# KrishnaswamyLab/MELD

Hardware: AMD Instinct MI355X
Metric: cells/sec through MELD.fit_transform (kNN+Chebyshev) (higher is better)
Workload: dtype f64

## Files before the change

include/meld_hip.h:

```cpp
#ifndef MELD_HIP_H
#define MELD_HIP_H

#include <stddef.h>
#include <stdint.h>

#ifdef __cplusplus
extern "C" {
#endif

#define MELD_OK 0
#define MELD_ERR_INVALID (-1)
#define MELD_ERR_UNSUPPORTED (-2)
#define MELD_ERR_HIP (-3)

typedef void* meld_stream_t;

int meld_abi_version(void);
const char* meld_last_error(void);
int meld_device_count(void);


int meld_knn_padded_dim(int d);
int meld_knn_tile_refs(void);
int meld_knn_block_queries(void);
// ... 274 lines not shown
                       const double* state, double* nrm2, meld_stream_t stream);
int meld_scale_f64(const double* x, double a, double* r, int64_t n, meld_stream_t stream);
int meld_axpby_f64(double a, const double* x, double b, double* y, int64_t n, double* nrm2,
                   meld_stream_t stream);

typedef struct meld_pt_layout {
  const int32_t* blk_row;
  const int32_t* blk_ntile;
  const int32_t* blk_ndist;
  const int32_t* seg;
  const int32_t* list_cols;
  const double* pval;
  const uint32_t* pidx;
  int32_t nb;
  const float* pval32;
  int64_t stream_len;
  const uint16_t* cdesc;
} meld_pt_layout_t;
int meld_pt_geometry(int* consumer_waves, int* rows_max, int* tile_cols, int* tiles_max);
int meld_pt_num_blocks(int64_t n_rows);
int64_t meld_pt_seg_len(int nb);
int64_t meld_pt_stream_len(int64_t nnz, int nb);
int64_t meld_pt_desc_len(int nb);
int meld_pt_build(const int64_t* rowptr, const int32_t* col, const double* val, int64_t n_rows, int64_t n_cols,
                  int64_t col_base, int symmetric, const meld_pt_layout_t* layout,
                  uint32_t* codes , int32_t* status, meld_stream_t stream);

int meld_rccl_available(void);
int meld_rccl_unique_id(void* id_host);
int meld_rccl_comm_create(const void* id_host, int world, int rank, void** comm);
int meld_rccl_comm_destroy(void* comm);
int meld_rccl_all_gather(void* comm, const void* send, void* recv, size_t bytes_per_rank, meld_stream_t stream);
int meld_rccl_all_reduce_sum_f64(void* comm, double* buf, size_t count, meld_stream_t stream);
int meld_cheby_run(void* comm, const meld_laplacian_t* L, int64_t rows_pad, int64_t row_begin, int p, double* t_a, double* t_b,
                   double* r, const double* coeffs, int n_coef, double alpha2, double beta2, int* last, meld_stream_t stream);
int meld_lanczos_steps_sharded(void* comm, const meld_laplacian_t* L, int64_t rows_pad, int64_t row_begin, double* v0, double* v1,
                               double* v2, double* state, double* acc, double* alphas, double* betas, int it_begin, int n_iter,
                               meld_stream_t stream);

int meld_kmeans_max_blocks(void);
int meld_kmeans_assign(const double* X, int64_t n, int d, const double* centroids, int k, int32_t* labels,
                       double* part_sum, double* part_cnt, double* part_inertia, int n_blocks, meld_stream_t stream);

int meld_kmeans_wide_max_d(void);
int meld_kmeans_wide_max_k(void);
int meld_kmeans_wide_assign(const double* Y, int64_t ldy, int64_t n, int d, const double* centres, int k, double* centre_norms,
// ... 141 lines not shown
```

meld_amd/_lib.py:

```python
from __future__ import annotations

from ._options import is_set, opt

import ctypes as C
import os

_HERE = os.path.dirname(os.path.abspath(__file__))
LIB_NAME = "libmeld_hip.so"
LIB_PATH = os.path.join(_HERE, LIB_NAME)

_i32, _i64, _f64, _sz, _ptr = C.c_int, C.c_int64, C.c_double, C.c_size_t, C.c_void_p

SIGNATURES = {
    "meld_abi_version": (_i32, []),
    "meld_last_error": (C.c_char_p, []),
    "meld_device_count": (_i32, []),
    "meld_knn_padded_dim": (_i32, [_i32]),
    "meld_knn_tile_refs": (_i32, []),
    "meld_knn_block_queries": (_i32, []),
    "meld_knn_row_capacity": (_i32, [_i32]),
    "meld_col_sums_f64": (_i32, [_ptr, _i64, _i32, _ptr, _ptr]),
    "meld_col_stats_temp_bytes": (_sz, [_i32]),
    "meld_col_stats_f64": (_i32, [_ptr, _i64, _i32, _ptr, _ptr, _ptr, _ptr, _sz, _ptr]),
    "meld_knn_prepare_refs": (_i32, [_ptr, _i64, _i32, _ptr, _i32, _ptr, _ptr, _ptr, _ptr]),
# ... 94 lines not shown
    "meld_csr_rows_sort_merge_sums": (_i32, [_ptr, _i64, _ptr, _ptr, _ptr, _ptr, _i32, _f64, _f64, _ptr, _ptr]),
    "meld_csr_compact_rows_anisotropy": (_i32, [_ptr, _i64, _ptr, _ptr, _ptr, _ptr, _ptr, _f64, _ptr, _ptr]),
    "meld_csr_compact_rows_sums": (_i32, [_ptr, _i64, _ptr, _ptr, _ptr, _ptr, _f64, _ptr, _ptr]),
    "meld_csr_row_sums": (_i32, [_ptr, _ptr, _i64, _f64, _ptr, _ptr]),
    "meld_csr_anisotropy": (_i32, [_ptr, _ptr, _ptr, _i64, _ptr, _i64, _f64, _ptr]),
    "meld_csr_anisotropy_degrees": (_i32, [_ptr, _ptr, _ptr, _i64, _ptr, _i64, _f64, _ptr, _ptr]),
    "meld_extend_rows_temp_bytes": (_sz, [_i64, _i64]),
    "meld_extend_rows": (_i32, [_ptr, _ptr, _i64, _i64, _i64, _i64, _ptr, _ptr, _ptr, _ptr, _ptr, _sz, _ptr]),
    "meld_extend_apply": (_i32, [_ptr, _ptr, _ptr, _ptr, _i64, _ptr, _i64, _i32, _ptr, _ptr, _ptr]),
    "meld_spmm_dot_slots": (_i32, []),
    "meld_cheby_step": (_i32, [_ptr, _i32, _ptr, _i64, _ptr, _ptr, _ptr, _f64, _f64, _f64, _f64, _ptr, _ptr]),
    "meld_lanczos_steps": (_i32, [_ptr, _ptr, _ptr, _ptr, _ptr, _ptr, _ptr, _i32, _i32, _ptr, _ptr, _ptr]),
    "meld_lanczos_spmv": (_i32, [_ptr, _ptr, _i64, _ptr, _ptr, _ptr, _ptr, _ptr]),
    "meld_lanczos_alpha": (_i32, [_ptr, _ptr, _ptr, _ptr, _i32, _ptr]),
    "meld_lanczos_axpy": (_i32, [_ptr, _ptr, _i64, _ptr, _ptr, _ptr]),
    "meld_lanczos_beta": (_i32, [_ptr, _ptr, _ptr, _ptr, _i32, _ptr]),
    "meld_lanczos_fold": (_i32, [_ptr, _ptr, _ptr, _ptr, _i32, _ptr]),
    "meld_lanczos_axpy3": (_i32, [_ptr, _ptr, _ptr, _i64, _ptr, _ptr, _ptr]),
    "meld_pt_geometry": (_i32, [_ptr, _ptr, _ptr, _ptr]),
    "meld_pt_num_blocks": (_i32, [_i64]),
    "meld_pt_seg_len": (_i64, [_i32]),
    "meld_pt_stream_len": (_i64, [_i64, _i32]),
    "meld_pt_desc_len": (_i64, [_i32]),
    "meld_pt_build": (_i32, [_ptr, _ptr, _ptr, _i64, _i64, _i64, _i32, _ptr, _ptr, _ptr, _ptr]),
    "meld_cheby_step_wide": (_i32, [_ptr, _i32, _ptr, _i64, _ptr, _ptr, _f64, _f64, _f64, _ptr]),
    "meld_block_max_blocks": (_i32, []),
    "meld_block_gram_f64": (_i32, [_ptr, _i64, _ptr, _i64, _i64, _i32, _ptr, _i32, _ptr, _ptr]),
    "meld_block_rotate_f64": (_i32, [_ptr, _i64, _ptr, _i64, _i32, _ptr, _i64, _ptr]),
    "meld_block_residuals_f64": (_i32, [_ptr, _ptr, _i64, _ptr, _i64, _i32, _ptr, _i32, _ptr, _ptr]),
    "meld_kmeans_max_blocks": (_i32, []),
    "meld_kmeans_assign": (_i32, [_ptr, _i64, _i32, _ptr, _i32, _ptr, _ptr, _ptr, _ptr, _i32, _ptr]),
    "meld_kmeans_wide_max_d": (_i32, []),
    "meld_kmeans_wide_max_k": (_i32, []),
    "meld_kmeans_wide_assign": (_i32, [_ptr, _i64, _i64, _i32, _ptr, _i32, _ptr, _ptr, _ptr, _ptr]),
    "meld_kmeans_wide_sums": (_i32, [_ptr, _i64, _i64, _i32, _ptr, _ptr, _i32, _ptr, _ptr]),
    "meld_scale_f64": (_i32, [_ptr, _f64, _ptr, _i64, _ptr]),
    "meld_axpby_f64": (_i32, [_f64, _ptr, _f64, _ptr, _i64, _ptr, _ptr]),
    "meld_normalize_rows_l1": (_i32, [_ptr, _ptr, _i64, _i32, _ptr]),
    "meld_assign_nearest": (_i32, [_ptr, _i64, _i32, _ptr, _i32, _ptr, _ptr, _ptr, _ptr]),
    "meld_chain_order": (_i32, [_ptr, _i64, _i32, _i32, _ptr, _ptr]),
    "meld_gather_rows_f64": (_i32, [_ptr, _ptr, _i64, _i32, _ptr, _ptr]),
    "meld_frame_max_dims": (_i32, []),
    "meld_cov_sample_f64": (_i32, [_ptr, _i64, _i32, _ptr, _i64, _ptr, _ptr]),
    "meld_rotate_rows_f64": (_i32, [_ptr, _i64, _i32, _ptr, _ptr, _ptr, _ptr]),
    "meld_argsort_u32_temp_bytes": (_sz, [_i64]),
    "meld_argsort_u32": (_i32, [_ptr, _i64, _i32, _ptr, _ptr, _ptr, _sz, _ptr]),
# ... 109 lines not shown
```

meld_amd/csrc/spmm_tiled.hip:

```cpp
#include "common.hpp"

#include <algorithm>
#include <cstdlib>
#include <cstring>

namespace meld {
namespace pt {

constexpr int NW = 12;
constexpr int NL = 4;
constexpr int THREADS = 64 * (NW + NL);
constexpr int RMAX = 4080;
constexpr int SLOTS = RMAX / NW;
constexpr int RPAD = 4096;
constexpr int CP = 1024;
constexpr int CP_BITS = 10;
constexpr int NB = 4;
constexpr int TMAX = 61;
constexpr int SEGW = 64;
constexpr int SEGROWS = 2 * (NW + 1);
constexpr int QW = 8;
constexpr int PADCAP = 64;
constexpr int KMAX = 512;
constexpr int KSLACK = 32;
// ... 428 lines not shown
        d_yy += yv.v[c] * yv.v[c];
      }
      stg<P>(ys, row, a.ld, a.colofs, yv);
      if (a.r != nullptr) stg<P>(a.r, row, a.ld, a.colofs, rl_[q]);
    }
  }
  if (a.dots != nullptr) {
    d_yx = wave_sum(d_yx);
    d_yy = wave_sum(d_yy);
    if (lane == 0) {
      s_dot[0][w] = d_yx;
      s_dot[1][w] = d_yy;
    }
    __syncthreads();
    if (tid < 2) {
      double s = 0.0;
      for (int k = 0; k < NW + NL; ++k) s += s_dot[tid][k];
      atomicAdd(&a.dots[tid * DOT_SLOTS + (b % DOT_SLOTS)], s);
    }
  }
}


__global__ __launch_bounds__(1024) void pt_plan_kernel(const int64_t* __restrict__ rowptr, int64_t n_rows, int nb,
                                                       int32_t* __restrict__ blk_row) {
  const int64_t nnz = rowptr[n_rows];
  for (int b = threadIdx.x; b < nb; b += blockDim.x) {
    const int64_t target = (nnz / nb) * (b + 1) + ((nnz % nb) * (b + 1)) / nb;
    int64_t lo = 0, hi = n_rows;
    while (lo < hi) {
      const int64_t mid = (lo + hi) >> 1;
      if (rowptr[mid] < target) lo = mid + 1; else hi = mid;
    }
    blk_row[b + 1] = (int32_t)((b == nb - 1) ? n_rows : lo);
  }
  __syncthreads();
  if (threadIdx.x == 0) {
    int64_t prev = 0;
    blk_row[0] = 0;
    for (int b = 0; b < nb; ++b) {
      int64_t cut = blk_row[b + 1];
      const int64_t must = n_rows - (int64_t)(nb - 1 - b) * RMAX;
      cut = max(cut, must);
      cut = min(cut, prev + RMAX);
      cut = min(max(cut, prev), n_rows);
      blk_row[b + 1] = (int32_t)cut;
      prev = cut;
    }
  }
}

constexpr int W_ENTRY = 361, W_FAR = 754, W_ROW = 2840;
__global__ __launch_bounds__(256) void pt_row_weight_kernel(const int64_t* __restrict__ rowptr, const int32_t* __restrict__ col,
                                                            int64_t n_rows, int64_t col_base, int win, int32_t* __restrict__ w) {
  const int64_t i = ((int64_t)blockIdx.x * blockDim.x + threadIdx.x) >> 4;
  const int sub = threadIdx.x & 15;
  int far = 0;
  int64_t e0 = 0, e1 = 0;
  if (i < n_rows) {
    e0 = rowptr[i];
    e1 = rowptr[i + 1];
    const int64_t self = col_base + i;
    for (int64_t e = e0 + sub; e < e1; e += 16) {
      const int64_t dlt = (int64_t)col[e] - self;
      far += (dlt > win || dlt < -win) ? 1 : 0;
    }
  }
#pragma unroll
  for (int off = 8; off > 0; off >>= 1) far += __shfl_xor(far, off, 64);
  if (i < n_rows && sub == 0) {
    const int64_t v = (int64_t)W_ENTRY * (e1 - e0) + (int64_t)W_FAR * far + W_ROW;
    w[i] = (int32_t)min(v, (int64_t)0x3fffffff);
  }
}
__global__ __launch_bounds__(1024) void pt_plan_weighted_kernel(const int64_t* __restrict__ wpre, int64_t n_rows, int nb,
                                                                int32_t* __restrict__ blk_row) {
  const int64_t tot = wpre[n_rows];
  for (int b = threadIdx.x; b < nb; b += blockDim.x) {
    const int64_t target = (tot / nb) * (b + 1) + ((tot % nb) * (b + 1)) / nb;
    int64_t lo = 0, hi = n_rows;
    while (lo < hi) {
      const int64_t mid = (lo + hi) >> 1;
      if (wpre[mid] < target) lo = mid + 1; else hi = mid;
    }
    blk_row[b + 1] = (int32_t)((b == nb - 1) ? n_rows : lo);
  }
  __syncthreads();
  if (threadIdx.x == 0) {
    int64_t prev = 0;
    blk_row[0] = 0;
    for (int b = 0; b < nb; ++b) {
      int64_t cut = blk_row[b + 1];
      const int64_t must = n_rows - (int64_t)(nb - 1 - b) * RMAX;
      cut = max(cut, must);
      cut = min(cut, prev + RMAX);
      cut = min(max(cut, prev), n_rows);
      blk_row[b + 1] = (int32_t)cut;
      prev = cut;
    }
  }
}

__device__ __forceinline__ int block_exscan(int v, int* s_wave , int* total) {
  const int lane = threadIdx.x & 63, w = threadIdx.x >> 6;
  int inc = v;
#pragma unroll
  for (int off = 1; off < 64; off <<= 1) {
    const int t = __shfl_up(inc, off, 64);
    if (lane >= off) inc += t;
  }
  __syncthreads();
  if (lane == 63) s_wave[w] = inc;
  __syncthreads();
  if (threadIdx.x == 0) {
    int run = 0;
    for (int k = 0; k < THREADS / 64; ++k) {
      const int t = s_wave[k];
      s_wave[k] = run;
      run += t;
    }
    s_wave[THREADS / 64] = run;
  }
  __syncthreads();
  *total = s_wave[THREADS / 64];
  return s_wave[w] + inc - v;
}

constexpr int GW = 4;
constexpr int GPP = (BP / 32) / GW;
constexpr int GROUPS_MAX = TP_MAX * GPP;
constexpr int GPT = (GROUPS_MAX + THREADS - 1) / THREADS;

__device__ __forceinline__ uint64_t lanes_below(int l) { return ((uint64_t)1 << l) - 1; }

__global__ __launch_bounds__(THREADS) void pt_build_kernel(
    const int64_t* __restrict__ rowptr, const int32_t* __restrict__ col, int64_t n_cols, int64_t col_base, int sym,
    int nb, const int32_t* __restrict__ blk_row, int32_t* __restrict__ blk_ntile, int32_t* __restrict__ blk_ndist,
    int32_t* __restrict__ seg, uint16_t* __restrict__ cdesc, int32_t* __restrict__ list_cols, uint32_t* __restrict__ codes,
    int32_t* __restrict__ status) {
  __shared__ int16_t s_pmap[NPAN_MAX];
  __shared__ uint32_t s_bits[TP_MAX][BP / 32];
  __shared__ int32_t s_gpre[GROUPS_MAX + 1];
  __shared__ int16_t s_cpan[TP_MAX];
  __shared__ int32_t s_cnt[NW][SEGW];
  __shared__ int32_t s_nin[NW];
  __shared__ int s_scan[THREADS / 64 + 1];
  __shared__ int32_t s_rp[RMAX + 1];
  __shared__ int s_ord[SEGW];
  __shared__ int s_tmp[2][SEGW];
  __shared__ int32_t s_len[NW];

  const int tid = threadIdx.x;
  const int lane = tid & 63;
  const int w = tid >> 6;
  const int b = blockIdx.x;
  const int row0 = blk_row[b];
  const int nrows = blk_row[b + 1] - row0;
  const int64_t e0 = rowptr[row0];
  const int64_t e1 = rowptr[row0 + nrows];
  const int npan = (int)((n_cols + BP - 1) / BP);
  const int64_t cb0 = col_base + row0;
  auto in_block = [&](int c) { return sym && (uint64_t)((int64_t)c - cb0) < (uint64_t)nrows; };
  int32_t* segp = seg + (size_t)b * SEGROWS * SEGW;

  for (int i = tid; i < NPAN_MAX; i += THREADS) s_pmap[i] = 0;
  for (int i = tid; i < TP_MAX * (BP / 32); i += THREADS) (&s_bits[0][0])[i] = 0u;
  for (int i = tid; i < NW * SEGW; i += THREADS) (&s_cnt[0][0])[i] = 0;
  for (int i = tid; i <= nrows; i += THREADS) s_rp[i] = (int32_t)(rowptr[row0 + i] - e0);
  for (int i = tid; i < SEGROWS * SEGW; i += THREADS) segp[i] = 0;
  __syncthreads();
  auto write_header = [&](int T_, int ndist_) {
    int32_t* h = segp + (SEGROWS - 1) * SEGW;
    h[2] = row0;
    h[3] = nrows;
    h[4] = T_;
    h[5] = ndist_;
    h[6] = (int32_t)(uint32_t)((uint64_t)e0 & 0xFFFFFFFFu);
    h[7] = (int32_t)(uint32_t)((uint64_t)e0 >> 32);
  };
  if (nrows == 0 || e1 == e0) {
    if (tid == 0) {
      blk_ntile[b] = 0;
      blk_ndist[b] = 0;
      write_header(0, 0);
    }
    return;
  }

  constexpr int MU = 8;
  for (int64_t eb = e0 + tid; eb < e1; eb += (int64_t)MU * THREADS) {
    int c[MU];
#pragma unroll
// ... 19 lines not shown
      if (pn < NPAN_MAX) s_pmap[pn] = f[k] ? (int16_t)(pre++) : (int16_t)-1;
    }
    if (tid == 0) s_scan[0] = total;
  }
  __syncthreads();
  const int tp_all = s_scan[0];
  __syncthreads();

  constexpr int RU = 8;
  const int nmine = (w < NW && nrows > w) ? (nrows - w + NW - 1) / NW : 0;
  const int64_t elast = max(e1 - 1, e0);
  int curs = 0;
  int in_cur = 0;
  int dist_base = 0;
  bool bad_range = false, bad_diag = false;
  const int n_groups_p = max(1, (tp_all + TP_MAX - 1) / TP_MAX);
  for (int pg = 0; pg < n_groups_p; ++pg) {
  const int pbase = pg * TP_MAX;
  const int tp = min(TP_MAX, tp_all - pbase);
  auto panel_slot = [&](int c) -> int {
    const int ci = (int)s_pmap[c >> BP_BITS] - pbase;
    return ((unsigned)ci < (unsigned)TP_MAX) ? ci : -1;
  };
  if (pg > 0) {
    for (int i = tid; i < TP_MAX * (BP / 32); i += THREADS) (&s_bits[0][0])[i] = 0u;
  }
  for (int pn = tid; pn < npan; pn += THREADS) {
    const int ci = (int)s_pmap[pn] - pbase;
    if (s_pmap[pn] >= 0 && (unsigned)ci < (unsigned)TP_MAX) s_cpan[ci] = (int16_t)pn;
  }
  __syncthreads();

  for (int64_t eb = e0 + tid; eb < e1; eb += (int64_t)MU * THREADS) {
    int c[MU];
#pragma unroll
    for (int u = 0; u < MU; ++u) c[u] = col[min(eb + (int64_t)u * THREADS, e1 - 1)];
#pragma unroll
    for (int u = 0; u < MU; ++u) {
      if (in_block(c[u])) continue;
      const int ci = panel_slot(c[u]);
      if (ci >= 0) atomicOr(&s_bits[ci][(c[u] & (BP - 1)) >> 5], 1u << (c[u] & 31));
    }
  }
  __syncthreads();
  int ndist_g;
  {
    const int ngroups = tp * GPP;
    int cntk[GPT], c = 0;
#pragma unroll
// ... 116 lines not shown
          bad_range |= ipos > 0x1FFF;
          codes[e0 + off + lane] = ((uint32_t)T_IN << 26) | ((uint32_t)(ipos & 0x1FFF) << 13) | ((uint32_t)ilast << 12) | (uint32_t)cg;
        } else if (first && inb) {
          codes[e0 + off + lane] = ((uint32_t)T_SKIP << 26) | (uint32_t)(cg & 0xFFF);
        }
        curs += __builtin_amdgcn_ds_permute((head ? ch : 63) << 2, head ? runlen : 0);
        in_cur += __popcll(um);
        if (u == RU - 1) busy = ik[0] < nmine;
      }
    }
  }
  dist_base += ndist_g;
  __syncthreads();
  }
  const int ndist = dist_base;
  const int T = (ndist + CP - 1) / CP;
  if (w < NW) {
    if (__any(bad_range)) atomicMax(status, 4);
    if (__any(bad_diag)) atomicMax(status, 6);
    s_cnt[w][lane] = (lane < T) ? curs : 0;
    if (lane == 0) s_nin[w] = in_cur;
  }
  __syncthreads();
  if (tid == 0) {
    int* tot = s_tmp[0];
    int* srt = s_tmp[1];
    for (int t = 0; t < T; ++t) {
      int c = 0;
      for (int ow = 0; ow < NW; ++ow) c += s_cnt[ow][t];
      tot[t] = c;
      int k = t;
      while (k > 0 && tot[srt[k - 1]] < c) {
        srt[k] = srt[k - 1];
        --k;
      }
      srt[k] = t;
    }
    int hi = 0, lo = T - 1, j = 0;
    while (hi <= lo) {
      s_ord[j++] = srt[hi++];
      for (int k = 0; k < 2 && hi <= lo; ++k) s_ord[j++] = srt[lo--];
    }
    for (int jj = T; jj < SEGW; ++jj) s_ord[jj] = 0;
    blk_ntile[b] = T;
    blk_ndist[b] = ndist;
    write_header(T, ndist);
  }
  __syncthreads();
  if (tid < NW) {
    const int ow = tid;
    const int nin = s_nin[ow];
    const int n_in_chunks = (nin + 63) >> 6;
    int32_t* bounds = segp + ow * SEGW;
    int32_t* eoff = segp + (NW + 1 + ow) * SEGW;
    uint16_t* cd = cdesc + ((size_t)b * NW + ow) * (KMAX + KSLACK);
    int k = 0, pos = 0;
    for (; k < n_in_chunks && k < KMAX; ++k) cd[k] = 64;
    bool over = n_in_chunks > KMAX;
    for (int j = 0; j < T; ++j) {
      const int cnt = s_cnt[ow][s_ord[j]];
      eoff[j] = pos;
      const int nch = max(1, (cnt + 63) >> 6);
      for (int c = 0; c < nch; ++c) {
        const int n = min(64, cnt - 64 * c);
        if (k < KMAX) cd[k] = (uint16_t)(max(n, 0) | (c == 0 ? D_FIRST : 0) | (c == nch - 1 ? D_LAST : 0));
        else over = true;
        ++k;
      }
      pos += cnt;
    }
    eoff[T] = pos;
    for (int q = min(k, KMAX); q < KMAX + KSLACK; ++q) cd[q] = 0;
    eoff[62] = nin;
    eoff[63] = pos;
    bounds[62] = n_in_chunks | (min(k, KMAX) << 16);
    s_len[ow] = (n_in_chunks << 6) + pos;
    if (over) atomicMax(status, 4);
  }
  __syncthreads();
  if (tid == 0) {
    int run = 0;
    for (int ow = 0; ow < NW; ++ow) {
      segp[ow * SEGW + 63] = run;
      run += s_len[ow];
    }
  }
  if (w == NW) segp[NW * SEGW + lane] = s_ord[lane];
}

constexpr int FILL_CAP = 12288;
__device__ __forceinline__ uint64_t pair_hash(uint32_t i, uint32_t j, double v) {
  uint64_t h = ((uint64_t)i << 32 | j) * 0x9E3779B97F4A7C15ull;
  h ^= (uint64_t)__double_as_longlong(v) * 0xC2B2AE3D27D4EB4Full;
  h ^= h >> 29;
  h *= 0xBF58476D1CE4E5B9ull;
  h ^= h >> 32;
  return h;
}
__global__ __launch_bounds__(THREADS) void pt_fill_kernel(const int64_t* __restrict__ rowptr, const double* __restrict__ val,
                                                          const uint32_t* __restrict__ codes, const int32_t* __restrict__ blk_row,
                                                          const int32_t* __restrict__ blk_ntile, int32_t* __restrict__ seg,
                                                          double* __restrict__ pval, uint32_t* __restrict__ pidx) {
  __shared__ double s_val[FILL_CAP];
  __shared__ uint32_t s_idx[FILL_CAP];
  __shared__ int s_eoff[SEGW], s_inv[SEGW];
  const int tid = threadIdx.x, lane = tid & 63, wv = tid >> 6;
  const int b = blockIdx.x / NW, w = blockIdx.x % NW;
  const int T = blk_ntile[b];
  if (T < 0) return;
  const int row0 = blk_row[b];
  const int nrows = blk_row[b + 1] - row0;
  if (nrows == 0) return;
  const int32_t* segp = seg + (size_t)b * SEGROWS * SEGW;
  const int hdr = segp[w * SEGW + 62];
  const int n_in_chunks = hdr & 0xFFFF;
  const int soff = segp[w * SEGW + 63];
  const int64_t sbase = stream_base(rowptr, row0, b) + soff;
  if (tid < SEGW) {
    s_eoff[tid] = segp[(NW + 1 + w) * SEGW + tid];
    if (tid < T) s_inv[segp[NW * SEGW + tid]] = tid;
  }
  __syncthreads();
  const int nmine = (nrows > w) ? (nrows - w + NW - 1) / NW : 0;
  const int in_base = n_in_chunks << 6;
  const int total = in_base + s_eoff[63];
  uint64_t hsum = 0;
  for (int a0 = 0; a0 < total || a0 == 0; a0 += FILL_CAP) {
    const int span = min(FILL_CAP, total - a0);
    for (int i = tid; i < span; i += THREADS) {
      s_val[i] = 0.0;
      s_idx[i] = 0u;
    }
    __syncthreads();
    auto place = [&](uint32_t code, double v, int rl) __attribute__((always_inline)) {
      const int tl = (int)(code >> 26);
      int slot;
      uint32_t word;
      if (tl == T_SKIP) {
        if (a0 == 0) hsum -= pair_hash(code & 0xFFF, (uint32_t)rl, v);
        return;
      } else if (tl == T_IN) {
        const int g = (code >> 13) & 0x1FFF;
        const int win = g / (64 * QW), u = g - win * (64 * QW);
        const int qw = min(QW, n_in_chunks - win * QW);
        const int l = u / qw, c = u - l * qw;
        slot = win * (64 * QW) + c * 64 + l;
        const uint32_t flush = ((code >> 12) & 1u) | (uint32_t)(c == qw - 1);
        const uint32_t rj = code & 0xFFF;
        word = flush | ((uint32_t)row_slot((int)rj) << 4) | ((uint32_t)row_slot(rl) << 20);
        if (a0 == 0) hsum += pair_hash((uint32_t)rl, rj, v);
      } else {
        const int j = s_inv[tl];
        const int pos = (int)((code >> CP_BITS) & 0x7FFF);
        const int n = s_eoff[j + 1] - s_eoff[j];
        const int q = n >> 6, r = n & 63;
        int l, c, mine;
        if (pos < r * (q + 1)) {
          l = pos / (q + 1);
          c = pos - l * (q + 1);
          mine = q + 1;
        } else {
          const int jj = pos - r * (q + 1);
          const int lq = jj / max(q, 1);
          l = r + lq;
          c = jj - lq * q;
          mine = q;
        }
        slot = in_base + s_eoff[j] + c * 64 + l;
        const uint32_t flush = ((code >> 25) & 1u) | (uint32_t)(c == mine - 1);
        const uint32_t cs = (uint32_t)((j & (NB - 1)) * CP) + (code & (CP - 1));
        word = flush | (cs << 4) | ((uint32_t)row_slot(rl) << 20);
      }
      slot -= a0;
      if (slot >= 0 && slot < span) {
        s_val[slot] = v;
        s_idx[slot] = word;
      }
    };
    constexpr int FG = 4;
    for (int k0 = wv; k0 < nmine; k0 += 16 * FG) {
      uint32_t code[FG];
      double v[FG];
      int64_t rs[FG], rend[FG];
#pragma unroll
      for (int g = 0; g < FG; ++g) {
        const int k = k0 + 16 * g;
        const int rl = w + min(k, nmine - 1) * NW;
        rs[g] = rowptr[row0 + rl];
        rend[g] = (k < nmine) ? rowptr[row0 + rl + 1] : rs[g];
        const int64_t e = min(rs[g] + lane, max(rend[g] - 1, rs[g]));
        code[g] = codes[e];
        v[g] = val[e];
      }
#pragma unroll
      for (int g = 0; g < FG; ++g) {
        const int rl = w + (k0 + 16 * g) * NW;
        if (rs[g] + lane < rend[g]) place(code[g], v[g], rl);
        for (int64_t e = rs[g] + 64 + lane; e < rend[g]; e += 64) place(codes[e], val[e], rl);
      }
    }
    __syncthreads();
    for (int i = tid; i < span; i += THREADS) {
      pval[sbase + a0 + i] = s_val[i];
      pidx[sbase + a0 + i] = s_idx[i];
    }
    __syncthreads();
  }
#pragma unroll
  for (int off = 32; off > 0; off >>= 1) hsum += __shfl_xor((unsigned long long)hsum, off, 64);
  if (lane == 0 && hsum != 0) atomicAdd(symsum_of(seg, b), (unsigned long long)hsum);
}

__global__ __launch_bounds__(256) void pt_symcheck_kernel(int32_t* __restrict__ seg, int nb, int32_t* __restrict__ status) {
  const int b = blockIdx.x * blockDim.x + threadIdx.x;
  if (b < nb && *symsum_of(seg, b) != 0ull) atomicMax(status, 5);
}

__global__ __launch_bounds__(256) void pt_round_f32_kernel(const double* __restrict__ pval, float* __restrict__ pval32, int64_t n) {
  for (int64_t i = ((int64_t)blockIdx.x * blockDim.x + threadIdx.x) * 2; i < n; i += (int64_t)gridDim.x * blockDim.x * 2) {
    if (i + 1 < n) {
      const double2 v = *reinterpret_cast<const double2*>(pval + i);
      *reinterpret_cast<float2*>(pval32 + i) = make_float2((float)v.x, (float)v.y);
    } else {
      pval32[i] = (float)pval[i];
    }
  }
}

}
}

using namespace meld;

extern "C" int meld_pt_geometry(int* consumer_waves, int* rows_max, int* tile_cols, int* tiles_max) {
  if (consumer_waves) *consumer_waves = pt::NW;
  if (rows_max) *rows_max = pt::RMAX;
  if (tile_cols) *tile_cols = pt::CP;
  if (tiles_max) *tiles_max = pt::TMAX;
  return MELD_OK;
}

extern "C" int meld_pt_num_blocks(int64_t n_rows) {
  if (n_rows <= 0) return 0;
  const int64_t target = (int64_t)(0.9576 * pt::RMAX);
  if (n_rows <= 64 * 256) return (int)std::max<int64_t>(1, ceil_div(n_rows, 256));
  const int64_t k = ceil_div(n_rows, 256 * target);
  int64_t nb = 256 * k;
  if (k == 1) nb = std::min<int64_t>(256, std::max<int64_t>(64, ceil_div(n_rows, 256)));
  while (nb * pt::RMAX < n_rows) nb += 256;
  return (int)nb;
}

extern "C" int64_t meld_pt_seg_len(int nb) { return (int64_t)nb * pt::SEGROWS * pt::SEGW; }
extern "C" int64_t meld_pt_desc_len(int nb) { return (int64_t)nb * pt::NW * (pt::KMAX + pt::KSLACK); }

extern "C" int64_t meld_pt_stream_len(int64_t nnz, int nb) {
  return nnz + (int64_t)nb * pt::NW * pt::PADCAP + (int64_t)(pt::U + 1) * 64;
}

extern "C" int meld_pt_build(const int64_t* rowptr, const int32_t* col, const double* val, int64_t n_rows, int64_t n_cols,
                             int64_t col_base, int symmetric, const meld_pt_layout_t* layout, uint32_t* codes,
                             int32_t* status, meld_stream_t stream) {
  MELD_CHECK_ARG(rowptr && col && val && layout && layout->blk_row && layout->blk_ntile && layout->blk_ndist && layout->seg &&
                     layout->list_cols && layout->pval && layout->pidx && layout->cdesc && codes && status && n_rows > 0 && layout->nb > 0 &&
                     n_cols > 0 && layout->stream_len > 0 && col_base >= 0,
                 "meld_pt_build: bad arguments");
  const int nb = layout->nb;
  MELD_CHECK_ARG((int64_t)nb * pt::RMAX >= n_rows, "meld_pt_build: %d blocks of %d rows cannot hold %lld rows", nb, pt::RMAX,
                 (long long)n_rows);
  hipStream_t st = S(stream);
  MELD_HIP_CALL(hipMemsetAsync(status, 0, sizeof(int32_t), st));
  if (ceil_div(n_cols, pt::BP) > pt::NPAN_MAX) {
    static const int32_t three = 3;
    MELD_HIP_CALL(hipMemcpyAsync(status, &three, sizeof(int32_t), hipMemcpyHostToDevice, st));
    return MELD_OK;
  }
  int32_t* seg = const_cast<int32_t*>(layout->seg);
  {
    static const bool by_entries = meld_dev_getenv("MELD_PT_PLAN") && !strcmp(meld_dev_getenv("MELD_PT_PLAN"), "entries");
    const size_t scan_bytes = meld_scan_temp_bytes(n_rows);
    const size_t off_w = sizeof(int64_t) * (size_t)(n_rows + 1), off_t = (off_w + sizeof(int32_t) * (size_t)n_rows + 255) / 256 * 256;
    if (!by_entries && nb > 1 && off_t + scan_bytes <= sizeof(double) * (size_t)layout->stream_len) {
      char* scratch = reinterpret_cast<char*>(const_cast<double*>(layout->pval));
      int64_t* wpre = reinterpret_cast<int64_t*>(scratch);
      int32_t* w = reinterpret_cast<int32_t*>(scratch + off_w);
      const int win = (int)std::max<int64_t>(1, n_rows / nb / 2);
      hipLaunchKernelGGL(pt::pt_row_weight_kernel, dim3((unsigned)ceil_div(n_rows * 16, 256)), dim3(256), 0, st, rowptr, col, n_rows,
                         col_base, win, w);
      const int rc = meld_exclusive_scan_i32_i64(w, wpre, n_rows, scratch + off_t, scan_bytes, stream);
      if (rc != MELD_OK) return rc;
      hipLaunchKernelGGL(pt::pt_plan_weighted_kernel, dim3(1), dim3(1024), 0, st, wpre, n_rows, nb, const_cast<int32_t*>(layout->blk_row));
    } else {
      hipLaunchKernelGGL(pt::pt_plan_kernel, dim3(1), dim3(1024), 0, st, rowptr, n_rows, nb, const_cast<int32_t*>(layout->blk_row));
    }
  }
  hipLaunchKernelGGL(pt::pt_build_kernel, dim3(nb), dim3(pt::THREADS), 0, st, rowptr, col, n_cols, col_base, symmetric ? 1 : 0, nb,
                     layout->blk_row, const_cast<int32_t*>(layout->blk_ntile), const_cast<int32_t*>(layout->blk_ndist), seg,
                     const_cast<uint16_t*>(layout->cdesc), const_cast<int32_t*>(layout->list_cols), codes, status);
  hipLaunchKernelGGL(pt::pt_fill_kernel, dim3(nb * pt::NW), dim3(pt::THREADS), 0, st, rowptr, val, codes, layout->blk_row,
                     layout->blk_ntile, seg, const_cast<double*>(layout->pval), const_cast<uint32_t*>(layout->pidx));
  if (symmetric)
    hipLaunchKernelGGL(pt::pt_symcheck_kernel, dim3((unsigned)ceil_div(nb, 256)), dim3(256), 0, st, seg, nb, status);
  if (layout->pval32 != nullptr)
    hipLaunchKernelGGL(pt::pt_round_f32_kernel, dim3(2048), dim3(256), 0, st, layout->pval, const_cast<float*>(layout->pval32),
                       layout->stream_len);
  MELD_LAUNCH_CHECK("pt_build_kernel");
  return MELD_OK;
}

namespace {
template <int P, bool F32>
int pt_launch(const pt::StepArgs& a, hipStream_t st) {
  constexpr size_t lds = pt::LDS_BYTES;
  static bool configured[64] = {};
  int dev = 0;
  if (hipGetDevice(&dev) != hipSuccess || dev < 0 || dev >= 64) dev = 0;
  if (!configured[dev]) {
    hipError_t e = hipFuncSetAttribute(reinterpret_cast<const void*>(&pt::pt_step_kernel<P, F32>),
                                       hipFuncAttributeMaxDynamicSharedMemorySize, (int)lds);
    if (e != hipSuccess) {
      set_err("pt_step_kernel: cannot reserve %zu bytes of LDS: %s", lds, hipGetErrorString(e));
      return MELD_ERR_HIP;
    }
    configured[dev] = true;
  }
  const unsigned grid = (unsigned)(ceil_div(a.nb, 8) * 8);
  hipLaunchKernelGGL((pt::pt_step_kernel<P, F32>), dim3(grid), dim3(pt::THREADS), lds, st, a);
  return MELD_OK;
// ... 34 lines not shown
```

Before: 29.46 million.

## Streamline tiled-Laplacian build: fuse f32 rounding, parallelize tile ordering, cheapen fill

Reworks the pt_build pipeline. The separate f32 rounding pass is folded into pt_fill's write-out, and the build kernel converts the scratch region in place. The per-block tile sort and chunk-descriptor scan move from a single thread to whole-wave parallel rank and shuffle scans. pt_fill replaces integer divisions with magic-multiply, caches row bounds and tile info in LDS, zero-fills only padding slots, and clears LDS in 16-byte stores. The plan kernels share one helper that writes cuts to LDS. This removes one kernel launch, a full pass over the stream, and serial per-block work. The trade-off is more intricate index math and extra preconditions on alignment and slot coverage.

Measured after the change: 29.04 million. 1.4% lower.

```diff
diff --git a/include/meld_hip.h b/include/meld_hip.h
--- a/include/meld_hip.h
+++ b/include/meld_hip.h
@@ -320,6 +320,7 @@
 int64_t meld_pt_seg_len(int nb);
 int64_t meld_pt_stream_len(int64_t nnz, int nb);
 int64_t meld_pt_desc_len(int nb);
+int meld_pt_fill_capacity(void);
 int meld_pt_build(const int64_t* rowptr, const int32_t* col, const double* val, int64_t n_rows, int64_t n_cols,
                   int64_t col_base, int symmetric, const meld_pt_layout_t* layout,
                   uint32_t* codes , int32_t* status, meld_stream_t stream);
diff --git a/meld_amd/_lib.py b/meld_amd/_lib.py
--- a/meld_amd/_lib.py
+++ b/meld_amd/_lib.py
@@ -140,6 +140,7 @@
     "meld_pt_seg_len": (_i64, [_i32]),
     "meld_pt_stream_len": (_i64, [_i64, _i32]),
     "meld_pt_desc_len": (_i64, [_i32]),
+    "meld_pt_fill_capacity": (_i32, []),
     "meld_pt_build": (_i32, [_ptr, _ptr, _ptr, _i64, _i64, _i64, _i32, _ptr, _ptr, _ptr, _ptr]),
     "meld_cheby_step_wide": (_i32, [_ptr, _i32, _ptr, _i64, _ptr, _ptr, _f64, _f64, _f64, _ptr]),
     "meld_block_max_blocks": (_i32, []),
diff --git a/meld_amd/csrc/spmm_tiled.hip b/meld_amd/csrc/spmm_tiled.hip
--- a/meld_amd/csrc/spmm_tiled.hip
+++ b/meld_amd/csrc/spmm_tiled.hip
@@ -474,32 +474,41 @@
 }
 
 
-__global__ __launch_bounds__(1024) void pt_plan_kernel(const int64_t* __restrict__ rowptr, int64_t n_rows, int nb,
-                                                       int32_t* __restrict__ blk_row) {
-  const int64_t nnz = rowptr[n_rows];
+constexpr int PLAN_LDS = 4096;
+__device__ __forceinline__ void plan_blocks(const int64_t* __restrict__ prefix, int64_t n_rows, int nb, int32_t* __restrict__ blk_row) {
+  __shared__ int32_t s_cut[PLAN_LDS];
+  int32_t* cuts = (nb <= PLAN_LDS) ? s_cut : blk_row + 1;
+  const int64_t tot = prefix[n_rows];
   for (int b = threadIdx.x; b < nb; b += blockDim.x) {
-    const int64_t target = (nnz / nb) * (b + 1) + ((nnz % nb) * (b + 1)) / nb;
+    const int64_t target = (tot / nb) * (b + 1) + ((tot % nb) * (b + 1)) / nb;
     int64_t lo = 0, hi = n_rows;
     while (lo < hi) {
       const int64_t mid = (lo + hi) >> 1;
-      if (rowptr[mid] < target) lo = mid + 1; else hi = mid;
-    }
-    blk_row[b + 1] = (int32_t)((b == nb - 1) ? n_rows : lo);
+      if (prefix[mid] < target) lo = mid + 1; else hi = mid;
+    }
+    cuts[b] = (int32_t)((b == nb - 1) ? n_rows : lo);
   }
   __syncthreads();
   if (threadIdx.x == 0) {
     int64_t prev = 0;
     blk_row[0] = 0;
     for (int b = 0; b < nb; ++b) {
-      int64_t cut = blk_row[b + 1];
+      int64_t cut = cuts[b];
       const int64_t must = n_rows - (int64_t)(nb - 1 - b) * RMAX;
       cut = max(cut, must);
       cut = min(cut, prev + RMAX);
       cut = min(max(cut, prev), n_rows);
-      blk_row[b + 1] = (int32_t)cut;
+      cuts[b] = (int32_t)cut;
       prev = cut;
     }
   }
+  __syncthreads();
+  if (nb <= PLAN_LDS)
+    for (int b = threadIdx.x; b < nb; b += blockDim.x) blk_row[b + 1] = s_cut[b];
+}
+__global__ __launch_bounds__(1024) void pt_plan_kernel(const int64_t* __restrict__ rowptr, int64_t n_rows, int nb,
+                                                       int32_t* __restrict__ blk_row) {
+  plan_blocks(rowptr, n_rows, nb, blk_row);
 }
 
 constexpr int W_ENTRY = 361, W_FAR = 754, W_ROW = 2840;
@@ -527,30 +536,7 @@
 }
 __global__ __launch_bounds__(1024) void pt_plan_weighted_kernel(const int64_t* __restrict__ wpre, int64_t n_rows, int nb,
                                                                 int32_t* __restrict__ blk_row) {
-  const int64_t tot = wpre[n_rows];
-  for (int b = threadIdx.x; b < nb; b += blockDim.x) {
-    const int64_t target = (tot / nb) * (b + 1) + ((tot % nb) * (b + 1)) / nb;
-    int64_t lo = 0, hi = n_rows;
-    while (lo < hi) {
-      const int64_t mid = (lo + hi) >> 1;
-      if (wpre[mid] < target) lo = mid + 1; else hi = mid;
-    }
-    blk_row[b + 1] = (int32_t)((b == nb - 1) ? n_rows : lo);
-  }
-  __syncthreads();
-  if (threadIdx.x == 0) {
-    int64_t prev = 0;
-    blk_row[0] = 0;
-    for (int b = 0; b < nb; ++b) {
-      int64_t cut = blk_row[b + 1];
-      const int64_t must = n_rows - (int64_t)(nb - 1 - b) * RMAX;
-      cut = max(cut, must);
-      cut = min(cut, prev + RMAX);
-      cut = min(max(cut, prev), n_rows);
-      blk_row[b + 1] = (int32_t)cut;
-      prev = cut;
-    }
-  }
+  plan_blocks(wpre, n_rows, nb, blk_row);
 }
 
 __device__ __forceinline__ int block_exscan(int v, int* s_wave , int* total) {
@@ -589,12 +575,12 @@
     const int64_t* __restrict__ rowptr, const int32_t* __restrict__ col, int64_t n_cols, int64_t col_base, int sym,
     int nb, const int32_t* __restrict__ blk_row, int32_t* __restrict__ blk_ntile, int32_t* __restrict__ blk_ndist,
     int32_t* __restrict__ seg, uint16_t* __restrict__ cdesc, int32_t* __restrict__ list_cols, uint32_t* __restrict__ codes,
-    int32_t* __restrict__ status) {
-  __shared__ int16_t s_pmap[NPAN_MAX];
-  __shared__ uint32_t s_bits[TP_MAX][BP / 32];
+    int32_t* __restrict__ status, const double* __restrict__ plan_scratch, float* __restrict__ pval32, int64_t n_scratch) {
+  __shared__ __attribute__((aligned(16))) int16_t s_pmap[NPAN_MAX];
+  __shared__ __attribute__((aligned(16))) uint32_t s_bits[TP_MAX][BP / 32];
   __shared__ int32_t s_gpre[GROUPS_MAX + 1];
   __shared__ int16_t s_cpan[TP_MAX];
-  __shared__ int32_t s_cnt[NW][SEGW];
+  __shared__ __attribute__((aligned(16))) int32_t s_cnt[NW][SEGW];
   __shared__ int32_t s_nin[NW];
   __shared__ int s_scan[THREADS / 64 + 1];
   __shared__ int32_t s_rp[RMAX + 1];
@@ -615,11 +601,22 @@
   auto in_block = [&](int c) { return sym && (uint64_t)((int64_t)c - cb0) < (uint64_t)nrows; };
   int32_t* segp = seg + (size_t)b * SEGROWS * SEGW;
 
-  for (int i = tid; i < NPAN_MAX; i += THREADS) s_pmap[i] = 0;
-  for (int i = tid; i < TP_MAX * (BP / 32); i += THREADS) (&s_bits[0][0])[i] = 0u;
-  for (int i = tid; i < NW * SEGW; i += THREADS) (&s_cnt[0][0])[i] = 0;
+  for (int64_t i = (int64_t)b * THREADS + tid; i < n_scratch; i += (int64_t)nb * THREADS) pval32[i] = (float)plan_scratch[i];
+
+  const uint4 zero4 = make_uint4(0u, 0u, 0u, 0u);
+  auto clear16 = [&](void* p, int bytes) {
+    for (int i = tid; i < bytes / 16; i += THREADS) reinterpret_cast<uint4*>(p)[i] = zero4;
+  };
+  static_assert(sizeof(s_pmap) % 16 == 0 && sizeof(s_bits) % 16 == 0 && sizeof(s_cnt) % 16 == 0 && (SEGROWS * SEGW * 4) % 16 == 0, "clear16");
+  clear16(s_pmap, (int)sizeof(s_pmap));
+  clear16(s_bits, (int)sizeof(s_bits));
+  clear16(s_cnt, (int)sizeof(s_cnt));
   for (int i = tid; i <= nrows; i += THREADS) s_rp[i] = (int32_t)(rowptr[row0 + i] - e0);
-  for (int i = tid; i < SEGROWS * SEGW; i += THREADS) segp[i] = 0;
+  if ((reinterpret_cast<uintptr_t>(segp) & 15) == 0) {
+    clear16(segp, SEGROWS * SEGW * 4);
+  } else {
+    for (int i = tid; i < SEGROWS * SEGW; i += THREADS) segp[i] = 0;
+  }
   __syncthreads();
   auto write_header = [&](int T_, int ndist_) {
     int32_t* h = segp + (SEGROWS - 1) * SEGW;
@@ -685,9 +682,7 @@
     const int ci = (int)s_pmap[c >> BP_BITS] - pbase;
     return ((unsigned)ci < (unsigned)TP_MAX) ? ci : -1;
   };
-  if (pg > 0) {
-    for (int i = tid; i < TP_MAX * (BP / 32); i += THREADS) (&s_bits[0][0])[i] = 0u;
-  }
+  if (pg > 0) clear16(s_bits, (int)sizeof(s_bits));
   for (int pn = tid; pn < npan; pn += THREADS) {
     const int ci = (int)s_pmap[pn] - pbase;
     if (s_pmap[pn] >= 0 && (unsigned)ci < (unsigned)TP_MAX) s_cpan[ci] = (int16_t)pn;
@@ -850,73 +845,83 @@
     if (lane == 0) s_nin[w] = in_cur;
   }
   __syncthreads();
-  if (tid == 0) {
+  if (w == 0) {
     int* tot = s_tmp[0];
     int* srt = s_tmp[1];
-    for (int t = 0; t < T; ++t) {
-      int c = 0;
-      for (int ow = 0; ow < NW; ++ow) c += s_cnt[ow][t];
-      tot[t] = c;
-      int k = t;
-      while (k > 0 && tot[srt[k - 1]] < c) {
-        srt[k] = srt[k - 1];
-        --k;
-      }
-      srt[k] = t;
-    }
-    int hi = 0, lo = T - 1, j = 0;
-    while (hi <= lo) {
-      s_ord[j++] = srt[hi++];
-      for (int k = 0; k < 2 && hi <= lo; ++k) s_ord[j++] = srt[lo--];
-    }
-    for (int jj = T; jj < SEGW; ++jj) s_ord[jj] = 0;
-    blk_ntile[b] = T;
-    blk_ndist[b] = ndist;
-    write_header(T, ndist);
-  }
-  __syncthreads();
-  if (tid < NW) {
-    const int ow = tid;
+    int c = 0;
+    if (lane < T)
+      for (int ow = 0; ow < NW; ++ow) c += s_cnt[ow][lane];
+    tot[lane] = c;
+    PT_WAIT_LDS();
+    __builtin_amdgcn_wave_barrier();
+    if (lane < T) {
+      int before = 0;
+      for (int t = 0; t < T; ++t) before += (tot[t] > c || (tot[t] == c && t < lane)) ? 1 : 0;
+      srt[before] = lane;
+    }
+    PT_WAIT_LDS();
+    __builtin_amdgcn_wave_barrier();
+    const int g3 = lane / 3, m3 = lane - 3 * g3;
+    s_ord[lane] = (lane < T) ? srt[m3 == 0 ? g3 : T - 1 - (2 * g3 + m3 - 1)] : 0;
+    if (lane == 0) {
+      blk_ntile[b] = T;
+      blk_ndist[b] = ndist;
+      write_header(T, ndist);
+    }
+  }
+  __syncthreads();
+  if (w < NW) {
+    const int ow = w;
     const int nin = s_nin[ow];
     const int n_in_chunks = (nin + 63) >> 6;
     int32_t* bounds = segp + ow * SEGW;
     int32_t* eoff = segp + (NW + 1 + ow) * SEGW;
     uint16_t* cd = cdesc + ((size_t)b * NW + ow) * (KMAX + KSLACK);
-    int k = 0, pos = 0;
-    for (; k < n_in_chunks && k < KMAX; ++k) cd[k] = 64;
-    bool over = n_in_chunks > KMAX;
-    for (int j = 0; j < T; ++j) {
-      const int cnt = s_cnt[ow][s_ord[j]];
-      eoff[j] = pos;
-      const int nch = max(1, (cnt + 63) >> 6);
+    const int k_in = min(n_in_chunks, KMAX);
+    for (int k = lane; k < k_in; k += 64) cd[k] = 64;
+    const int cnt = (lane < T) ? s_cnt[ow][s_ord[lane]] : 0;
+    const int nch = (lane < T) ? max(1, (cnt + 63) >> 6) : 0;
+    int kend = nch, pend = cnt;
+#pragma unroll
+    for (int off = 1; off < 64; off <<= 1) {
+      const int tk = __shfl_up(kend, off, 64), tp = __shfl_up(pend, off, 64);
+      if (lane >= off) {
+        kend += tk;
+        pend += tp;
+      }
+    }
+    const int k_all = k_in + __shfl(kend, 63, 64);
+    const int pos = __shfl(pend, 63, 64);
+    if (lane < T) {
+      eoff[lane] = pend - cnt;
+      const int k0 = k_in + kend - nch;
       for (int c = 0; c < nch; ++c) {
         const int n = min(64, cnt - 64 * c);
-        if (k < KMAX) cd[k] = (uint16_t)(max(n, 0) | (c == 0 ? D_FIRST : 0) | (c == nch - 1 ? D_LAST : 0));
-        else over = true;
-        ++k;
-      }
-      pos += cnt;
-    }
-    eoff[T] = pos;
-    for (int q = min(k, KMAX); q < KMAX + KSLACK; ++q) cd[q] = 0;
-    eoff[62] = nin;
-    eoff[63] = pos;
-    bounds[62] = n_in_chunks | (min(k, KMAX) << 16);
-    s_len[ow] = (n_in_chunks << 6) + pos;
-    if (over) atomicMax(status, 4);
-  }
-  __syncthreads();
-  if (tid == 0) {
+        if (k0 + c < KMAX) cd[k0 + c] = (uint16_t)(max(n, 0) | (c == 0 ? D_FIRST : 0) | (c == nch - 1 ? D_LAST : 0));
+      }
+    }
+    for (int q = min(k_all, KMAX) + lane; q < KMAX + KSLACK; q += 64) cd[q] = 0;
+    if (lane == 0) {
+      eoff[T] = pos;
+      eoff[62] = nin;
+      eoff[63] = pos;
+      bounds[62] = n_in_chunks | (min(k_all, KMAX) << 16);
+      s_len[ow] = (n_in_chunks << 6) + pos;
+      if (n_in_chunks > KMAX || k_all > KMAX) atomicMax(status, 4);
+    }
+  }
+  __syncthreads();
+  if (tid < NW) {
     int run = 0;
-    for (int ow = 0; ow < NW; ++ow) {
-      segp[ow * SEGW + 63] = run;
-      run += s_len[ow];
-    }
+    for (int ow = 0; ow < tid; ++ow) run += s_len[ow];
+    segp[tid * SEGW + 63] = run;
   }
   if (w == NW) segp[NW * SEGW + lane] = s_ord[lane];
 }
 
 constexpr int FILL_CAP = 12288;
+__device__ __forceinline__ uint32_t div_magic(int d) { return d < 2 ? 0u : 0xFFFFFFFFu / (uint32_t)d + 1u; }
+__device__ __forceinline__ int div_by(int x, uint32_t magic) { return magic ? (int)__umulhi((uint32_t)x, magic) : x; }
 __device__ __forceinline__ uint64_t pair_hash(uint32_t i, uint32_t j, double v) {
   uint64_t h = ((uint64_t)i << 32 | j) * 0x9E3779B97F4A7C15ull;
   h ^= (uint64_t)__double_as_longlong(v) * 0xC2B2AE3D27D4EB4Full;
@@ -928,10 +933,12 @@
 __global__ __launch_bounds__(THREADS) void pt_fill_kernel(const int64_t* __restrict__ rowptr, const double* __restrict__ val,
                                                           const uint32_t* __restrict__ codes, const int32_t* __restrict__ blk_row,
                                                           const int32_t* __restrict__ blk_ntile, int32_t* __restrict__ seg,
-                                                          double* __restrict__ pval, uint32_t* __restrict__ pidx) {
+                                                          double* __restrict__ pval, uint32_t* __restrict__ pidx,
+                                                          float* __restrict__ pval32) {
   __shared__ double s_val[FILL_CAP];
   __shared__ uint32_t s_idx[FILL_CAP];
-  __shared__ int s_eoff[SEGW], s_inv[SEGW];
+  __shared__ int4 s_tile[SEGW];
+  __shared__ int s_rs[SLOTS], s_re[SLOTS];
   const int tid = threadIdx.x, lane = tid & 63, wv = tid >> 6;
   const int b = blockIdx.x / NW, w = blockIdx.x % NW;
   const int T = blk_ntile[b];
@@ -939,68 +946,86 @@
   const int row0 = blk_row[b];
   const int nrows = blk_row[b + 1] - row0;
   if (nrows == 0) return;
+  const int64_t e0 = rowptr[row0], e1 = rowptr[row0 + nrows];
+  if (e1 == e0) return;
   const int32_t* segp = seg + (size_t)b * SEGROWS * SEGW;
   const int hdr = segp[w * SEGW + 62];
   const int n_in_chunks = hdr & 0xFFFF;
   const int soff = segp[w * SEGW + 63];
-  const int64_t sbase = stream_base(rowptr, row0, b) + soff;
-  if (tid < SEGW) {
-    s_eoff[tid] = segp[(NW + 1 + w) * SEGW + tid];
-    if (tid < T) s_inv[segp[NW * SEGW + tid]] = tid;
-  }
-  __syncthreads();
+  const int nin = segp[(NW + 1 + w) * SEGW + 62];
+  const int in_base = n_in_chunks << 6;
+  const int total = in_base + segp[(NW + 1 + w) * SEGW + 63];
+  const int64_t sbase = e0 + (int64_t)b * (NW * PADCAP) + soff;
   const int nmine = (nrows > w) ? (nrows - w + NW - 1) / NW : 0;
-  const int in_base = n_in_chunks << 6;
-  const int total = in_base + s_eoff[63];
+  if (tid < nmine) {
+    const int rl = w + tid * NW;
+    s_rs[tid] = (int)(rowptr[row0 + rl] - e0);
+    s_re[tid] = (int)(rowptr[row0 + rl + 1] - e0);
+  }
+  if (tid < T) {
+    const int tl = segp[NW * SEGW + tid];
+    const int eo = segp[(NW + 1 + w) * SEGW + tid];
+    const int n = segp[(NW + 1 + w) * SEGW + tid + 1] - eo;
+    const int q = n >> 6;
+    s_tile[tl] = make_int4(in_base + eo, n | ((tid & (NB - 1)) << 16), (int)div_magic(q + 1), (int)div_magic(q));
+  }
+  const int wlast = max((n_in_chunks + QW - 1) / QW - 1, 0) * (64 * QW);
+  const int qw_last = max(n_in_chunks - wlast / 64, 1);
+  const uint32_t mq_last = 0xFFFFu / (uint32_t)qw_last + 1u;
+  __syncthreads();
   uint64_t hsum = 0;
   for (int a0 = 0; a0 < total || a0 == 0; a0 += FILL_CAP) {
     const int span = min(FILL_CAP, total - a0);
-    for (int i = tid; i < span; i += THREADS) {
-      s_val[i] = 0.0;
-      s_idx[i] = 0u;
-    }
-    __syncthreads();
-    auto place = [&](uint32_t code, double v, int rl) __attribute__((always_inline)) {
+    for (int s = wlast + tid; s < in_base; s += THREADS) {
+      const int u = s & (64 * QW - 1);
+      const int gpos = s - u + (u & 63) * qw_last + (u >> 6);
+      const int slot = s - a0;
+      if (gpos >= nin && (unsigned)slot < (unsigned)span) {
+        s_val[slot] = 0.0;
+        s_idx[slot] = 0u;
+      }
+    }
+    auto place = [&](uint32_t code, double v, int k) __attribute__((always_inline)) {
       const int tl = (int)(code >> 26);
+      const int rl = w + k * NW;
+      const uint32_t rword = (uint32_t)(w * SLOTS + k) << 20;
       int slot;
       uint32_t word;
-      if (tl == T_SKIP) {
-        if (a0 == 0) hsum -= pair_hash(code & 0xFFF, (uint32_t)rl, v);
-        return;
-      } else if (tl == T_IN) {
+      if (tl >= T_SKIP) {
+        static_assert(T_SKIP == 62 && T_IN == 63, "the two in-block markers are the two largest codes");
+        const bool skip = tl == T_SKIP;
+        const uint32_t rj = code & 0xFFF;
+        if (a0 == 0) {
+          const uint64_t h = pair_hash(skip ? rj : (uint32_t)rl, skip ? (uint32_t)rl : rj, v);
+          hsum += skip ? (uint64_t)0 - h : h;
+        }
+        if (skip) return;
         const int g = (code >> 13) & 0x1FFF;
-        const int win = g / (64 * QW), u = g - win * (64 * QW);
-        const int qw = min(QW, n_in_chunks - win * QW);
-        const int l = u / qw, c = u - l * qw;
-        slot = win * (64 * QW) + c * 64 + l;
+        const int wbase = g & ~(64 * QW - 1), u = g - wbase;
+        const bool lastw = wbase == wlast;
+        const int qw = lastw ? qw_last : QW;
+        const int l = (int)(((uint32_t)u * (lastw ? mq_last : (0x10000u / QW))) >> 16), c = u - l * qw;
+        slot = wbase + c * 64 + l;
         const uint32_t flush = ((code >> 12) & 1u) | (uint32_t)(c == qw - 1);
-        const uint32_t rj = code & 0xFFF;
-        word = flush | ((uint32_t)row_slot((int)rj) << 4) | ((uint32_t)row_slot(rl) << 20);
-        if (a0 == 0) hsum += pair_hash((uint32_t)rl, rj, v);
+        word = flush | ((uint32_t)row_slot((int)rj) << 4) | rword;
       } else {
-        const int j = s_inv[tl];
+        const int4 ti = s_tile[tl];
         const int pos = (int)((code >> CP_BITS) & 0x7FFF);
-        const int n = s_eoff[j + 1] - s_eoff[j];
+        const int n = ti.y & 0xFFFF;
         const int q = n >> 6, r = n & 63;
-        int l, c, mine;
-        if (pos < r * (q + 1)) {
-          l = pos / (q + 1);
-          c = pos - l * (q + 1);
-          mine = q + 1;
-        } else {
-          const int jj = pos - r * (q + 1);
-          const int lq = jj / max(q, 1);
-          l = r + lq;
-          c = jj - lq * q;
-          mine = q;
-        }
-        slot = in_base + s_eoff[j] + c * 64 + l;
+        const bool head = pos < r * (q + 1);
+        const int x = head ? pos : pos - r * (q + 1);
+        const int mine = head ? q + 1 : q;
+        const int lq = div_by(x, (uint32_t)(head ? ti.z : ti.w));
+        const int l = head ? lq : r + lq;
+        const int c = x - lq * mine;
+        slot = ti.x + c * 64 + l;
         const uint32_t flush = ((code >> 25) & 1u) | (uint32_t)(c == mine - 1);
-        const uint32_t cs = (uint32_t)((j & (NB - 1)) * CP) + (code & (CP - 1));
-        word = flush | (cs << 4) | ((uint32_t)row_slot(rl) << 20);
+        const uint32_t cs = (uint32_t)((ti.y >> 16) * CP) + (code & (CP - 1));
+        word = flush | (cs << 4) | rword;
       }
       slot -= a0;
-      if (slot >= 0 && slot < span) {
+      if ((unsigned)slot < (unsigned)span) {
         s_val[slot] = v;
         s_idx[slot] = word;
       }
@@ -1009,28 +1034,37 @@
     for (int k0 = wv; k0 < nmine; k0 += 16 * FG) {
       uint32_t code[FG];
       double v[FG];
-      int64_t rs[FG], rend[FG];
+      int rs[FG], rend[FG];
 #pragma unroll
       for (int g = 0; g < FG; ++g) {
         const int k = k0 + 16 * g;
-        const int rl = w + min(k, nmine - 1) * NW;
-        rs[g] = rowptr[row0 + rl];
-        rend[g] = (k < nmine) ? rowptr[row0 + rl + 1] : rs[g];
-        const int64_t e = min(rs[g] + lane, max(rend[g] - 1, rs[g]));
+        const int kk = min(k, nmine - 1);
+        rs[g] = s_rs[kk];
+        rend[g] = (k < nmine) ? s_re[kk] : rs[g];
+        const int64_t e = min(e0 + min(rs[g] + lane, max(rend[g] - 1, rs[g])), e1 - 1);
         code[g] = codes[e];
         v[g] = val[e];
       }
 #pragma unroll
       for (int g = 0; g < FG; ++g) {
-        const int rl = w + (k0 + 16 * g) * NW;
-        if (rs[g] + lane < rend[g]) place(code[g], v[g], rl);
-        for (int64_t e = rs[g] + 64 + lane; e < rend[g]; e += 64) place(codes[e], val[e], rl);
+        const int k = k0 + 16 * g;
+        if (rs[g] + lane < rend[g]) place(code[g], v[g], k);
+        for (int e = rs[g] + 64 + lane; e < rend[g]; e += 64) place(codes[e0 + e], val[e0 + e], k);
       }
     }
     __syncthreads();
-    for (int i = tid; i < span; i += THREADS) {
-      pval[sbase + a0 + i] = s_val[i];
-      pidx[sbase + a0 + i] = s_idx[i];
+    if (pval32 != nullptr) {
+      for (int i = tid; i < span; i += THREADS) {
+        const double v = s_val[i];
+        pval[sbase + a0 + i] = v;
+        pidx[sbase + a0 + i] = s_idx[i];
+        pval32[sbase + a0 + i] = (float)v;
+      }
+    } else {
+      for (int i = tid; i < span; i += THREADS) {
+        pval[sbase + a0 + i] = s_val[i];
+        pidx[sbase + a0 + i] = s_idx[i];
+      }
     }
     __syncthreads();
   }
@@ -1042,17 +1076,6 @@
 __global__ __launch_bounds__(256) void pt_symcheck_kernel(int32_t* __restrict__ seg, int nb, int32_t* __restrict__ status) {
   const int b = blockIdx.x * blockDim.x + threadIdx.x;
   if (b < nb && *symsum_of(seg, b) != 0ull) atomicMax(status, 5);
-}
-
-__global__ __launch_bounds__(256) void pt_round_f32_kernel(const double* __restrict__ pval, float* __restrict__ pval32, int64_t n) {
-  for (int64_t i = ((int64_t)blockIdx.x * blockDim.x + threadIdx.x) * 2; i < n; i += (int64_t)gridDim.x * blockDim.x * 2) {
-    if (i + 1 < n) {
-      const double2 v = *reinterpret_cast<const double2*>(pval + i);
-      *reinterpret_cast<float2*>(pval32 + i) = make_float2((float)v.x, (float)v.y);
-    } else {
-      pval32[i] = (float)pval[i];
-    }
-  }
 }
 
 }
@@ -1067,6 +1090,8 @@
   if (tiles_max) *tiles_max = pt::TMAX;
   return MELD_OK;
 }
+
+extern "C" int meld_pt_fill_capacity(void) { return pt::FILL_CAP; }
 
 extern "C" int meld_pt_num_blocks(int64_t n_rows) {
   if (n_rows <= 0) return 0;
@@ -1104,6 +1129,7 @@
     return MELD_OK;
   }
   int32_t* seg = const_cast<int32_t*>(layout->seg);
+  int64_t n_scratch = 0;
   {
     static const bool by_entries = meld_dev_getenv("MELD_PT_PLAN") && !strcmp(meld_dev_getenv("MELD_PT_PLAN"), "entries");
     const size_t scan_bytes = meld_scan_temp_bytes(n_rows);
@@ -1118,20 +1144,20 @@
       const int rc = meld_exclusive_scan_i32_i64(w, wpre, n_rows, scratch + off_t, scan_bytes, stream);
       if (rc != MELD_OK) return rc;
       hipLaunchKernelGGL(pt::pt_plan_weighted_kernel, dim3(1), dim3(1024), 0, st, wpre, n_rows, nb, const_cast<int32_t*>(layout->blk_row));
+      if (layout->pval32 != nullptr) n_scratch = (int64_t)ceil_div((int64_t)(off_t + scan_bytes), (int64_t)sizeof(double));
     } else {
       hipLaunchKernelGGL(pt::pt_plan_kernel, dim3(1), dim3(1024), 0, st, rowptr, n_rows, nb, const_cast<int32_t*>(layout->blk_row));
     }
   }
   hipLaunchKernelGGL(pt::pt_build_kernel, dim3(nb), dim3(pt::THREADS), 0, st, rowptr, col, n_cols, col_base, symmetric ? 1 : 0, nb,
                      layout->blk_row, const_cast<int32_t*>(layout->blk_ntile), const_cast<int32_t*>(layout->blk_ndist), seg,
-                     const_cast<uint16_t*>(layout->cdesc), const_cast<int32_t*>(layout->list_cols), codes, status);
+                     const_cast<uint16_t*>(layout->cdesc), const_cast<int32_t*>(layout->list_cols), codes, status, layout->pval,
+                     const_cast<float*>(layout->pval32), n_scratch);
   hipLaunchKernelGGL(pt::pt_fill_kernel, dim3(nb * pt::NW), dim3(pt::THREADS), 0, st, rowptr, val, codes, layout->blk_row,
-                     layout->blk_ntile, seg, const_cast<double*>(layout->pval), const_cast<uint32_t*>(layout->pidx));
+                     layout->blk_ntile, seg, const_cast<double*>(layout->pval), const_cast<uint32_t*>(layout->pidx),
+                     const_cast<float*>(layout->pval32));
   if (symmetric)
     hipLaunchKernelGGL(pt::pt_symcheck_kernel, dim3((unsigned)ceil_div(nb, 256)), dim3(256), 0, st, seg, nb, status);
-  if (layout->pval32 != nullptr)
-    hipLaunchKernelGGL(pt::pt_round_f32_kernel, dim3(2048), dim3(256), 0, st, layout->pval, const_cast<float*>(layout->pval32),
-                       layout->stream_len);
   MELD_LAUNCH_CHECK("pt_build_kernel");
   return MELD_OK;
 }
```
